# GlassyWing/yolo_deepsort

Measured on AMD Instinct MI355X. Metric: end-to-end frames/sec (detect+ReID+assoc), 608x608, higher is better.
Workload: dtype f16x3

## Files before the change

yolo_deepsort_amd/csrc/conv_f16x3.hip:

```cpp
#include "conv_common.h"

#include <map>
#include <mutex>

#include <math.h>
#include <string.h>

namespace yds {


constexpr int ROWB = 144;
__device__ __forceinline__ void split4(const f32x4 &v, h4 &hi, h4 &lo) {
#pragma unroll
    for (int c = 0; c < 4; ++c) {
        float xs = v[c] * A_SCALE;
        _Float16 h = (_Float16)xs;
        hi[c] = h;
        lo[c] = (_Float16)((xs - (float)h) * LO_SCALE);
    }
}

template <int BM, int BN, int ACT, int RES, int AIN>
__global__ __launch_bounds__(256, 2) void conv_igemm_f16x3(ConvKernelArgs p) {
    fp16_saturate_on();
    constexpr int WM = 2, WN = 2;
    constexpr int TM = BM / WM / 32, TN = BN / WN / 32;
    constexpr int A_ROWS = BM / 32, B_ROWS = BN / 32;
    extern __shared__ __attribute__((aligned(16))) char smem16[];
    char *As = smem16;
    char *Bs = smem16 + 2 * BM * ROWB;

    const int tid = threadIdx.x;
    const int lane = tid & 63, wave = __builtin_amdgcn_readfirstlane(tid >> 6);
    const int wm = wave / WN, wn = wave % WN;
    int m0, n0;
    {
        int tm, tn;
        if (!tile_of_block(p, tm, tn)) return;
        m0 = tm * BM;
        n0 = tn * BN;
    }
    const int cq = tid & 7;
    const int r0 = tid >> 3;

    int a_base[A_ROWS], a_iy[A_ROWS], a_ix[A_ROWS];
    const int HoWo = p.Ho * p.Wo;
#pragma unroll
    for (int i = 0; i < A_ROWS; ++i) {
        int m = m0 + r0 + 32 * i;
        if (m < p.M) {
            int img = m / HoWo, rem = m - img * HoWo;
            int oy = rem / p.Wo, ox = rem - oy * p.Wo;
            a_iy[i] = oy * p.stride - p.pad;
            a_ix[i] = ox * p.stride - p.pad;
            a_base[i] = ((img * p.H + a_iy[i]) * p.W + a_ix[i]) * p.ldx;
        } else {
            a_iy[i] = -(1 << 28);
            a_ix[i] = 0;
            a_base[i] = 0;
        }
    }
    int kk = cq * 4, kh = 0, kw = 0, kc = AIN == FMT_H16 ? 0 : kk;
    if (AIN != FMT_H16)
        while (kc >= p.Cin) { kc -= p.Cin; if (++kw == p.ksize) { kw = 0; ++kh; } }
    unsigned w_off[B_ROWS];
#pragma unroll
    for (int i = 0; i < B_ROWS; ++i) w_off[i] = (unsigned)min(n0 + r0 + 32 * i, p.Cout - 1) * (unsigned)p.Kpad * 4u + cq * 16;
    const char *w_bytes = reinterpret_cast<const char *>(p.w), *x_bytes = reinterpret_cast<const char *>(p.x);

    f32x4 a_reg[A_ROWS], b_reg[B_ROWS];
    unsigned a_ok = 0, a_off[A_ROWS], tap_ok = 0;
    int kt_load = 0;
    auto set_tap = [&]() {
        tap_ok = 0;
#pragma unroll
        for (int i = 0; i < A_ROWS; ++i) {
            int iy = a_iy[i] + kh, ix = a_ix[i] + kw;
            bool ok = (unsigned)iy < (unsigned)p.H && (unsigned)ix < (unsigned)p.W;
            tap_ok |= (ok ? 1u : 0u) << i;
            a_off[i] = ok ? (unsigned)(a_base[i] + (kh * p.W + kw) * p.ldx + cq * 4) * 4u : cq * 16u;
        }
    };
    if (AIN == FMT_H16) set_tap();
    auto load_tiles = [&]() {
        if (AIN == FMT_H16) {
            a_ok = tap_ok;
            const char *xg = x_bytes + (size_t)kc * 4;
#pragma unroll
            for (int i = 0; i < A_ROWS; ++i) a_reg[i] = *reinterpret_cast<const f32x4 *>(xg + a_off[i]);
        } else {
            const int tap_off = (kh * p.W + kw) * p.ldx + kc;
            const bool k_ok = kk < p.K;
            a_ok = 0;
#pragma unroll
            for (int i = 0; i < A_ROWS; ++i) {
                int iy = a_iy[i] + kh, ix = a_ix[i] + kw;
                bool ok = k_ok && (unsigned)iy < (unsigned)p.H && (unsigned)ix < (unsigned)p.W;
                a_ok |= (ok ? 1u : 0u) << i;
                a_reg[i] = *reinterpret_cast<const f32x4 *>(p.x + (ok ? a_base[i] + tap_off : 0));
            }
        }
        const char *wg = w_bytes + (size_t)kt_load * 128;
#pragma unroll
        for (int i = 0; i < B_ROWS; ++i) b_reg[i] = *reinterpret_cast<const f32x4 *>(wg + w_off[i]);
    };
    auto advance_k = [&]() {
        ++kt_load;
        kk += 32;
        kc += 32;
        if (AIN == FMT_H16) {
            if (kc >= p.Cin) { kc = 0; if (++kw == p.ksize) { kw = 0; ++kh; } set_tap(); }
        } else {
            while (kc >= p.Cin) { kc -= p.Cin; if (++kw == p.ksize) { kw = 0; ++kh; } }
        }
    };
    auto store_tiles = [&](int buf) {
        char *a = As + buf * BM * ROWB, *b = Bs + buf * BN * ROWB;
#pragma unroll
        for (int i = 0; i < A_ROWS; ++i) {
            f32x4 v = a_reg[i];
            if (!((a_ok >> i) & 1u)) v = f32x4{0, 0, 0, 0};
            if (AIN == FMT_H16) {
                *reinterpret_cast<f32x4 *>(a + (r0 + 32 * i) * ROWB + cq * 16) = v;
            } else {
                h4 hi, lo;
                split4(v, hi, lo);
                char *row = a + (r0 + 32 * i) * ROWB + cq * 8;
                *reinterpret_cast<h4 *>(row) = hi;
                *reinterpret_cast<h4 *>(row + 64) = lo;
            }
        }
#pragma unroll
        for (int i = 0; i < B_ROWS; ++i) *reinterpret_cast<f32x4 *>(b + (r0 + 32 * i) * ROWB + cq * 16) = b_reg[i];
    };

    f32x16 acc1[TM][TN], acc2[TM][TN];
#pragma unroll
    for (int i = 0; i < TM; ++i)
#pragma unroll
        for (int j = 0; j < TN; ++j)
#pragma unroll
            for (int e = 0; e < 16; ++e) { acc1[i][j][e] = 0.f; acc2[i][j][e] = 0.f; }

    const int nk = p.Kpad / 32;
    load_tiles();
    store_tiles(0);
    if (STAGGER && ((blockIdx.x >> 8) & 1)) __builtin_amdgcn_s_sleep(STAGGER / 4);
    __syncthreads();

    const int frag_off = (lane & 31) * ROWB + (lane >> 5) * 16;
    const char *a_lds = As + wm * (BM / WM) * ROWB + frag_off;
    const char *b_lds = Bs + wn * (BN / WN) * ROWB + frag_off;
    for (int kt = 0; kt < nk; ++kt) {
        const int cur = kt & 1;
        const bool more = kt + 1 < nk;
        if (more) { advance_k(); load_tiles(); }
        const char *a = a_lds + cur * BM * ROWB, *b = b_lds + cur * BN * ROWB;
#pragma unroll
        for (int s = 0; s < 2; ++s) {
            h8 ah[TM], al[TM], bh[TN], bl[TN];
#pragma unroll
            for (int i = 0; i < TM; ++i) {
                ah[i] = *reinterpret_cast<const h8 *>(a + i * 32 * ROWB + s * 32);
                al[i] = *reinterpret_cast<const h8 *>(a + i * 32 * ROWB + s * 32 + 64);
            }
#pragma unroll
            for (int j = 0; j < TN; ++j) {
                bh[j] = *reinterpret_cast<const h8 *>(b + j * 32 * ROWB + s * 32);
                bl[j] = *reinterpret_cast<const h8 *>(b + j * 32 * ROWB + s * 32 + 64);
            }
#pragma unroll
            for (int i = 0; i < TM; ++i)
#pragma unroll
                for (int j = 0; j < TN; ++j) {
                    acc1[i][j] = __builtin_amdgcn_mfma_f32_32x32x16_f16(ah[i], bh[j], acc1[i][j], 0, 0, 0);
                    acc2[i][j] = __builtin_amdgcn_mfma_f32_32x32x16_f16(ah[i], bl[j], acc2[i][j], 0, 0, 0);
                    acc2[i][j] = __builtin_amdgcn_mfma_f32_32x32x16_f16(al[i], bh[j], acc2[i][j], 0, 0, 0);
                }
        }
        if (more) store_tiles(cur ^ 1);
        __syncthreads();
    }
#pragma unroll
    for (int i = 0; i < TM; ++i)
#pragma unroll
        for (int j = 0; j < TN; ++j)
#pragma unroll
            for (int e = 0; e < 16; ++e) acc1[i][j][e] = (acc1[i][j][e] + acc2[i][j][e] * (1.f / LO_SCALE)) * (1.f / A_SCALE);
    static_assert(BM * (BN + 4) * 4 <= 2 * (BM + BN) * ROWB, "whole-tile epilogue staging must fit the main-loop LDS");
    conv_epilogue<BM, BN, WM, WN, ACT, RES, BM / WM / 32, BN / WN / 32, 256, true>(p, acc1, reinterpret_cast<float *>(smem16), m0, n0, tid);
}


constexpr int ZERO_PAGE_BYTES = 64 * 1024;

constexpr size_t dma_smem_bytes(int BM, int BN, int NS) {
    return (size_t)NS * (BM + BN) * 128 > conv_stage_bytes(BM, BN) ? (size_t)NS * (BM + BN) * 128 : conv_stage_bytes(BM, BN);
}
template <int BM, int BN, int WM, int WN, int NS, int ACT, int RES, int TERMS>
__global__ __launch_bounds__(WM * WN * 64, (WM * WN != 4 || dma_smem_bytes(BM, BN, NS) > 80 * 1024) ? 1 : (dma_smem_bytes(BM, BN, NS) <= 53 * 1024 ? 3 : 2))
void conv_igemm_f16x3_dma(ConvKernelArgs p, const char *zero_page) {
    fp16_saturate_on();
    constexpr int NW = WM * WN, NT = NW * 64;
    constexpr int TM = BM / WM / 32, TN = BN / WN / 32;
    constexpr int ROW = 128;
    constexpr int A_BYTES = BM * ROW, STAGE = (BM + BN) * ROW;
    constexpr int A_INST = BM / (8 * NW), B_INST = BN / (8 * NW);
    constexpr int IN = A_INST + B_INST;
    static_assert(NS >= 2 && NS <= 4 && A_INST >= 1 && B_INST >= 1, "ring shape");
    extern __shared__ __attribute__((aligned(16))) char ring[];

    const int tid = threadIdx.x;
    const int lane = tid & 63, wave = __builtin_amdgcn_readfirstlane(tid >> 6);
    const int wm = wave / WN, wn = wave % WN;
    int m0, n0;
    {
        int tm, tn;
        if (!tile_of_block(p, tm, tn)) return;
        m0 = tm * BM;
        n0 = tn * BN;
    }
    const int drow = lane >> 3, dpos = lane & 7;
    int a_base[A_INST], a_iy[A_INST], a_ix[A_INST];
    const char *a_src[A_INST];
    const int HoWo = p.Ho * p.Wo;
#pragma unroll
    for (int q = 0; q < A_INST; ++q) {
        const int row = (q * NW + wave) * 8 + drow;
        const int m = m0 + row;
        if (m < p.M) {
            int img = m / HoWo, rem = m - img * HoWo;
            int oy = rem / p.Wo, ox = rem - oy * p.Wo;
            a_iy[q] = oy * p.stride - p.pad;
            a_ix[q] = ox * p.stride - p.pad;
            a_base[q] = ((img * p.H + a_iy[q]) * p.W + a_ix[q]) * p.ldx;
        } else {
            a_iy[q] = -(1 << 28);
            a_ix[q] = 0;
            a_base[q] = 0;
        }
    }
    constexpr int KC = TERMS == 4 ? 64 : 32;
    const bool xs = TERMS == 4 && p.fmt_x == FMT_F16;
    const int xbpc = xs ? 2 : 4;
    auto src_chunk = [&](int q, bool act) {
        const int c = dpos ^ ((((q * NW + wave) * 8 + drow) >> 1) & 7);
        return ((TERMS == 4 && !(act && xs)) ? ((c >> 2) << 3) + (c & 3) : c) * 16;
    };
    const char *w_src[B_INST];
#pragma unroll
    for (int q = 0; q < B_INST; ++q) {
        const int row = (q * NW + wave) * 8 + drow;
        w_src[q] = reinterpret_cast<const char *>(p.w) + (size_t)min(n0 + row, p.Cout - 1) * p.Kpad * 4 + src_chunk(q, false);
    }
    const int nk_all = p.K / KC;
    int t_begin = 0, nk = nk_all;
    if (gridDim.y > 1) {
        const int per = (nk_all + gridDim.y - 1) / gridDim.y;
        t_begin = blockIdx.y * per;
        nk = max(0, min(nk_all, t_begin + per) - t_begin);
        p.y += (size_t)blockIdx.y * (size_t)p.M * p.ldy;
    }
    const int kcs = p.Cin / KC;
    int kh = (t_begin / kcs) / p.ksize, kw = (t_begin / kcs) % p.ksize, kc = (t_begin % kcs) * KC;
#pragma unroll
    for (int q = 0; q < B_INST; ++q) w_src[q] += (size_t)t_begin * (KC * 4);
    auto set_tap = [&]() {
#pragma unroll
        for (int q = 0; q < A_INST; ++q) {
            int iy = a_iy[q] + kh, ix = a_ix[q] + kw;
            bool ok = (unsigned)iy < (unsigned)p.H && (unsigned)ix < (unsigned)p.W;
            a_src[q] = ok ? reinterpret_cast<const char *>(p.x + (a_base[q] + (kh * p.W + kw) * p.ldx)) + src_chunk(q, true) : zero_page;
        }
    };
    set_tap();
    auto piece = [&](int stage, int q) {
        char *sa = ring + stage * STAGE, *sb = sa + A_BYTES;
        if (q < A_INST) {
            __builtin_amdgcn_global_load_lds((glb_void_t *)(a_src[q] + kc * xbpc), (lds_void_t *)(sa + (q * NW + wave) * 8 * ROW), 16, 0, 0);
        } else {
            const int b = q - A_INST;
            __builtin_amdgcn_global_load_lds((glb_void_t *)w_src[b], (lds_void_t *)(sb + (b * NW + wave) * 8 * ROW), 16, 0, 0);
            w_src[b] += KC * 4;
        }
    };
    auto advance_tile = [&]() {
        kc += KC;
        if (kc >= p.Cin) { kc = 0; if (++kw == p.ksize) { kw = 0; ++kh; } set_tap(); }
    };

    f32x16 acc1[TM][TN], acc2[TM][TN];
#pragma unroll
    for (int i = 0; i < TM; ++i)
#pragma unroll
        for (int j = 0; j < TN; ++j)
#pragma unroll
            for (int e = 0; e < 16; ++e) { acc1[i][j][e] = 0.f; acc2[i][j][e] = 0.f; }

#pragma unroll
    for (int s = 0; s < NS - 1; ++s)
        if (s < nk) {
#pragma unroll
            for (int q = 0; q < IN; ++q) piece(s, q);
            advance_tile();
        }
    if (STAGGER && ((blockIdx.x >> 8) & 1)) __builtin_amdgcn_s_sleep(STAGGER / 4);

    const int swz = (lane >> 1) & 7, kb = lane >> 5;
    const int a_frag = (wm * (BM / WM) + (lane & 31)) * ROW, b_frag = A_BYTES + (wn * (BN / WN) + (lane & 31)) * ROW;
    int pos_hi[2], pos_lo[2];
#pragma unroll
    for (int s = 0; s < 2; ++s) { pos_hi[s] = ((2 * s + kb) ^ swz) * 16; pos_lo[s] = ((4 + 2 * s + kb) ^ swz) * 16; }

    constexpr int NF = 2 * (TM + TN);
    constexpr int NM = 3 * TM * TN;
    h8 fr[2][NF];
    auto frag_read = [&](const char *st, int s, int f) {
        const int which = f / 2, lo = f & 1;
        if (TERMS == 1 && lo) return;
        const int off = which < TM ? a_frag + which * 32 * ROW : b_frag + (which - TM) * 32 * ROW;
        fr[s][f] = *reinterpret_cast<const h8 *>(st + off + (lo ? pos_lo[s] : pos_hi[s]));
    };
    auto mfma = [&](int s, int m) {
        const int ij = m / 3, term = m % 3, i = ij / TN, j = ij % TN;
        if (TERMS == 1 && term != 0) return;
        const h8 ah = fr[s][2 * i], al = fr[s][2 * i + 1], bh = fr[s][2 * (TM + j)], bl = fr[s][2 * (TM + j) + 1];
        if (TERMS == 4) {
            if (term == 0) acc1[i][j] = __builtin_amdgcn_mfma_f32_32x32x16_f16(ah, bh, acc1[i][j], 0, 0, 0);
            else if (term == 1) acc1[i][j] = __builtin_amdgcn_mfma_f32_32x32x16_f16(al, bl, acc1[i][j], 0, 0, 0);
            return;
        }
        if (term == 0) acc1[i][j] = __builtin_amdgcn_mfma_f32_32x32x16_f16(ah, bh, acc1[i][j], 0, 0, 0);
        else if (term == 1) acc2[i][j] = __builtin_amdgcn_mfma_f32_32x32x16_f16(ah, bl, acc2[i][j], 0, 0, 0);
        else acc2[i][j] = __builtin_amdgcn_mfma_f32_32x32x16_f16(al, bh, acc2[i][j], 0, 0, 0);
    };
    constexpr int P0 = IN < NM - 4 ? IN : NM - 4;
    constexpr int F0 = NM - P0 < NF ? NM - P0 : NF;
    static_assert(IN - P0 + NF - F0 <= NM, "not enough MFMA slots for the interleaved memory instructions");
    auto frag_order = [&](int k) {
        if (k < 2) return k;
        if (k < 4) return 2 * TM + (k - 2);
        const int r = k - 4, nb = 2 * (TN - 1);
        return r < nb ? 2 * TM + 2 + r : 2 + (r - nb);
    };
    auto step = [&](int t, auto refill_c) {
        constexpr bool REFILL = decltype(refill_c)::value;
        const char *st = ring + (t % NS) * STAGE;
        const int fill_stage = (t + NS - 1) % NS;
#pragma unroll
        for (int f = 0; f < NF; ++f) frag_read(st, 0, f);
        __builtin_amdgcn_sched_barrier(0);
#pragma unroll
        for (int m = 0; m < NM; ++m) {
            mfma(0, m);
            __builtin_amdgcn_sched_barrier(0);
            if (m < P0) { if (REFILL) piece(fill_stage, m); }
            else if (m - P0 < F0) frag_read(st, 1, frag_order(m - P0));
            __builtin_amdgcn_sched_barrier(0);
        }
#pragma unroll
        for (int m = 0; m < NM; ++m) {
            mfma(1, m);
            __builtin_amdgcn_sched_barrier(0);
            if (m < NF - F0) frag_read(st, 1, frag_order(F0 + m));
            else if (REFILL && P0 + (m - (NF - F0)) < IN) piece(fill_stage, P0 + (m - (NF - F0)));
            __builtin_amdgcn_sched_barrier(0);
        }
        if (REFILL) advance_tile();
    };
    int t = 0;
    for (; t + NS - 1 < nk; ++t) {
        wait_vmcnt<(NS - 2) * IN>();
        __builtin_amdgcn_s_barrier();
        step(t, std::true_type{});
    }
    for (; t < nk; ++t) {
        const int younger = nk - 1 - t;
        if (younger >= 1 && NS >= 3) wait_vmcnt<(NS >= 3 ? IN : 0)>(); else wait_vmcnt<0>();
        __builtin_amdgcn_s_barrier();
        step(t, std::false_type{});
    }
    __syncthreads();
#pragma unroll
    for (int i = 0; i < TM; ++i)
#pragma unroll
        for (int j = 0; j < TN; ++j)
#pragma unroll
            for (int e = 0; e < 16; ++e)
                acc1[i][j][e] = TERMS != 3 ? acc1[i][j][e] * (1.f / A_SCALE) : (acc1[i][j][e] + acc2[i][j][e] * (1.f / LO_SCALE)) * (1.f / A_SCALE);
    conv_epilogue<BM, BN, WM, WN, ACT, RES, TM, TN, NT, true>(p, acc1, reinterpret_cast<float *>(ring), m0, n0, tid);
}

static const char *zero_page_dev() {
    static void *z = nullptr;
    if (!z) {
        YDS_HIP(hipMalloc(&z, ZERO_PAGE_BYTES));
        YDS_HIP(hipMemset(z, 0, ZERO_PAGE_BYTES));
    }
    return static_cast<const char *>(z);
}

template <int BM, int BN, int WM, int WN, int NS> static void launch_cfg_dma(const ConvKernelArgs &k, hipStream_t s) {
    const bool xs = k.fmt_x == FMT_F16;
    if (xs ? (k.terms != 1 || k.Cin % 64) : (k.fmt_x != FMT_H16 || k.Cin % 32)) fail("conv: the LDS-DMA kernel needs a pre-split (H16, or F16 in half mode) input");
    if ((size_t)k.Cin * 4 + 128 > (size_t)ZERO_PAGE_BYTES) fail("conv: %d input channels exceed the zero page of the LDS-DMA kernel", k.Cin);
    auto launch = [&](auto A, auto R, auto terms_c) {
        constexpr int TERMS = decltype(terms_c)::value;
        launch_conv_tiles<conv_igemm_f16x3_dma<BM, BN, WM, WN, NS, A, R, TERMS>>(k, BM, BN, k.ksplit > 1 ? k.ksplit : 1, WM * WN * 64, dma_smem_bytes(BM, BN, NS), s,
                                                                                  zero_page_dev());
    };
    dispatch_act_res(k, [&](auto A, auto R) {
        if (k.terms == 1 && k.Cin % 64 == 0) launch(A, R, std::integral_constant<int, 4>{});
        else if (k.terms == 1) launch(A, R, std::integral_constant<int, 1>{});
        else launch(A, R, std::integral_constant<int, 3>{});
    });
}

__global__ __launch_bounds__(256) void splitk_reduce_kernel(const float *ws, int ksplit, int M, int ldw, ConvKernelArgs p) {
    fp16_saturate_on();
    const int c4 = (p.Cout + 3) / 4;
    const int idx = blockIdx.x * 256 + threadIdx.x;
    if (idx >= M * c4) return;
    const int m = idx / c4, n = (idx - m * c4) * 4;
    float v[4] = {0.f, 0.f, 0.f, 0.f};
    for (int z = 0; z < ksplit; ++z) {
        const float4 t = *reinterpret_cast<const float4 *>(ws + ((size_t)z * M + m) * ldw + n);
        v[0] += t.x; v[1] += t.y; v[2] += t.z; v[3] += t.w;
    }
    float r[4] = {0.f, 0.f, 0.f, 0.f};
    const bool full = n + 3 < p.Cout;
    if (p.res_mode != RES_NONE) {
        const float *rp = p.res + (size_t)m * p.ldr;
        if (p.fmt_r == FMT_H16 || full) load4(rp, n, p.fmt_r, r);
        else for (int k = 0; k < 4; ++k) if (n + k < p.Cout) r[k] = rp[n + k];
    }
#pragma unroll
    for (int k = 0; k < 4; ++k) {
        float o = v[k] + (n + k < p.Cout ? p.bias[n + k] : 0.f);
        if (p.res_mode == RES_BEFORE_ACT) o += r[k];
        o = p.act == ACT_LEAKY ? apply_act<ACT_LEAKY>(o) : p.act == ACT_MISH ? apply_act<ACT_MISH>(o) : p.act == ACT_RELU ? apply_act<ACT_RELU>(o) : o;
        if (p.res_mode == RES_AFTER_ACT) o += r[k];
        v[k] = o;
    }
    float *yp = p.y + (size_t)m * p.ldy;
    if (p.fmt_y == FMT_H16 || full) store4(yp, n, p.fmt_y, v);
    else for (int k = 0; k < 4; ++k) if (n + k < p.Cout) yp[n + k] = v[k];
}

int conv_splitk_factor(const ConvKernelArgs &k, int BM, int BN) {
    const long tiles = (long)((k.M + BM - 1) / BM) * ((k.Cout + BN - 1) / BN);
    const int nk = k.K / 32;
    int s = (int)((512 + tiles - 1) / tiles);
    s = std::min(s, std::min(16, nk / 4));
    return s >= 2 ? s : 1;
}

static float *splitk_workspace(size_t floats, hipStream_t s) {
    static std::mutex mu;
    static std::map<hipStream_t, DevBuf<float>> bufs;
    std::lock_guard<std::mutex> lock(mu);
    DevBuf<float> &b = bufs[s];
    if (b.n < floats) {
        YDS_HIP(hipStreamSynchronize(s));
        b.alloc(floats + floats / 2);
    }
    return b.p;
}

template <int BM, int BN> static void launch_splitk(const ConvKernelArgs &k, hipStream_t s) {
    if (k.fmt_x != FMT_H16 || k.Cin % 32) fail("conv: the split-K LDS-DMA kernel needs a pre-split (H16) input");
    if ((size_t)k.Cout * 4 > (size_t)ZERO_PAGE_BYTES) fail("conv: %d filters exceed the zero page used as the split-K bias", k.Cout);
    const int ksplit = conv_splitk_factor(k, BM, BN);
    if (ksplit < 2) fail("conv: split-K does not apply (the layer already has enough tiles or too few K steps)");
    const int ldw = (k.Cout + 3) / 4 * 4;
    float *ws = splitk_workspace((size_t)ksplit * k.M * ldw, s);
    ConvKernelArgs part = k;
    part.y = ws; part.ldy = ldw; part.fmt_y = FMT_F32;
    part.bias = reinterpret_cast<const float *>(zero_page_dev());
    part.res = nullptr; part.res_mode = RES_NONE; part.fmt_r = FMT_F32; part.act = ACT_LINEAR;
    part.ksplit = ksplit;
    launch_cfg_dma<BM, BN, 2, 2, 2>(part, s);
    const int c4 = (k.Cout + 3) / 4;
    hipLaunchKernelGGL(splitk_reduce_kernel, dim3(((size_t)k.M * c4 + 255) / 256), dim3(256), 0, s, ws, ksplit, k.M, ldw, k);
    YDS_HIP(hipGetLastError());
}

bool conv_splitk_preferred(const ConvKernelArgs &k) {
    if (k.fmt_x != FMT_H16 || k.Cin % 32) return false;
    const long tiles = (long)((k.M + 63) / 64) * ((k.Cout + 127) / 128);
    return tiles <= 128 && k.K / 32 >= 32 && conv_splitk_factor(k, 64, 128) >= 2;
}

bool conv_splitk_applicable(const ConvKernelArgs &k, int tile) {
    if (k.fmt_x != FMT_H16 || k.Cin % 32) return false;
    return tile == 0 ? conv_splitk_factor(k, 64, 128) >= 2 : conv_splitk_factor(k, 128, 128) >= 2;
}

template <int BM, int BN> static void launch_cfg16(const ConvKernelArgs &k, hipStream_t s) {
    if (k.fmt_x == FMT_F16) fail("conv: the register-staged kernel does not read 2-byte (F16) activations");
    constexpr size_t smem = 2ull * (BM + BN) * ROWB;
    dispatch_act_res(k, [&](auto A, auto R) {
        if (k.fmt_x == FMT_H16) launch_conv_tiles<conv_igemm_f16x3<BM, BN, A, R, FMT_H16>>(k, BM, BN, 1, 256, smem, s);
        else launch_conv_tiles<conv_igemm_f16x3<BM, BN, A, R, FMT_F32>>(k, BM, BN, 1, 256, smem, s);
    });
}

void launch_conv_f16x3_staged(ConvKernelArgs k, int tile, hipStream_t s) {
    switch (tile) {
        case 0: launch_cfg16<128, 128>(k, s); break;
        case 1: launch_cfg16<64, 128>(k, s); break;
        case 2: launch_cfg16<128, 64>(k, s); break;
        default: launch_cfg16<64, 64>(k, s); break;
    }
}

void launch_conv_f16x3_dma(ConvKernelArgs k, int tile, hipStream_t s) {
    switch (tile) {
        case 0: launch_cfg_dma<128, 128, 2, 2, 2>(k, s); break;
        case 1: launch_cfg_dma<256, 128, 4, 2, 3>(k, s); break;
        case 2: launch_cfg_dma<128, 256, 2, 4, 3>(k, s); break;
        case 3: launch_cfg_dma<128, 128, 2, 2, 3>(k, s); break;
        case 4: launch_cfg_dma<128, 64, 2, 2, 2>(k, s); break;
        default: launch_cfg_dma<64, 128, 2, 2, 2>(k, s); break;
    }
}

void launch_conv_f16x3_win(ConvKernelArgs k, int tile, hipStream_t s) {
    if (!conv_win_applicable(k)) fail("conv: the window-resident kernel needs a 3x3 stride-1 layer with a pre-split input and W <= 95 (W <= 318 for 32 input channels)");
    if (k.terms == 1) launch_conv_win(k, tile, s);
    else launch_conv_win16(k, tile, s);
}

void launch_conv_f16x3_splitk(ConvKernelArgs k, int tile, hipStream_t s) {
    if (tile == 0) launch_splitk<64, 128>(k, s);
    else launch_splitk<128, 128>(k, s);
}

void pack_weights_f16x3(const float *w, int cout, int kpad, std::vector<uint16_t> &out) {
    out.assign((size_t)cout * kpad * 2, 0);
    for (int o = 0; o < cout; ++o)
        for (int k = 0; k < kpad; ++k) {
            float x = w[(size_t)o * kpad + k];
            if (!(fabsf(x) < 65504.f)) fail("conv: weight %g does not fit the fp16 split (|w| must be < 65504)", (double)x);
            _Float16 h = (_Float16)x;
            _Float16 l = (_Float16)((x - (float)h) * LO_SCALE);
            size_t base = ((size_t)o * (kpad / 32) + k / 32) * 64;
            uint16_t hb, lb;
            memcpy(&hb, &h, 2);
            memcpy(&lb, &l, 2);
            out[base + (k & 31)] = hb;
            out[base + 32 + (k & 31)] = lb;
        }
}

}
```

Baseline: 1649.

## Add 16x16x32 MFMA quadrant-pipelined body for f16x3 LDS-DMA conv kernel

For the three-term split-f16 path on selected tile shapes, this adds an alternative main loop built on 16x16x32 MFMAs in place of 32x32x16. The wave tile is split into quadrants, and the fragment reads and DMA refills are interleaved between quadrant MFMA groups. All NS stages are prefetched and there is one barrier per tile, placed mid-step. The goal is to hide LDS fragment reads and global-to-LDS loads more fully behind MFMA work. It relies on a conv_epilogue16 helper that is not shown here, and it raises register pressure and scheduling complexity.

```diff
diff --git a/yolo_deepsort_amd/csrc/conv_f16x3.hip b/yolo_deepsort_amd/csrc/conv_f16x3.hip
--- a/yolo_deepsort_amd/csrc/conv_f16x3.hip
+++ b/yolo_deepsort_amd/csrc/conv_f16x3.hip
@@ -197,6 +197,20 @@
 constexpr size_t dma_smem_bytes(int BM, int BN, int NS) {
     return (size_t)NS * (BM + BN) * 128 > conv_stage_bytes(BM, BN) ? (size_t)NS * (BM + BN) * 128 : conv_stage_bytes(BM, BN);
 }
+#ifndef YDS_DMA16
+#define YDS_DMA16 -1
+#endif
+constexpr bool dma_body16(int BM, int BN, int NS) {
+    if (YDS_DMA16 >= 0) return YDS_DMA16 != 0;
+    if (BM == 128 && BN == 128 && NS == 2) return true;
+    if (BM == 256 && BN == 128) return true;
+    if (BM == 128 && BN == 256) return true;
+    if (BM == 128 && BN == 128 && NS == 3) return false;
+    if (BM == 128 && BN == 64) return true;
+    if (BM == 64 && BN == 128) return true;
+    return false;
+}
+
 template <int BM, int BN, int WM, int WN, int NS, int ACT, int RES, int TERMS>
 __global__ __launch_bounds__(WM * WN * 64, (WM * WN != 4 || dma_smem_bytes(BM, BN, NS) > 80 * 1024) ? 1 : (dma_smem_bytes(BM, BN, NS) <= 53 * 1024 ? 3 : 2))
 void conv_igemm_f16x3_dma(ConvKernelArgs p, const char *zero_page) {
@@ -289,106 +303,250 @@
         if (kc >= p.Cin) { kc = 0; if (++kw == p.ksize) { kw = 0; ++kh; } set_tap(); }
     };
 
-    f32x16 acc1[TM][TN], acc2[TM][TN];
-#pragma unroll
-    for (int i = 0; i < TM; ++i)
-#pragma unroll
-        for (int j = 0; j < TN; ++j)
-#pragma unroll
-            for (int e = 0; e < 16; ++e) { acc1[i][j][e] = 0.f; acc2[i][j][e] = 0.f; }
-
-#pragma unroll
-    for (int s = 0; s < NS - 1; ++s)
-        if (s < nk) {
-#pragma unroll
-            for (int q = 0; q < IN; ++q) piece(s, q);
-            advance_tile();
-        }
-    if (STAGGER && ((blockIdx.x >> 8) & 1)) __builtin_amdgcn_s_sleep(STAGGER / 4);
-
-    const int swz = (lane >> 1) & 7, kb = lane >> 5;
-    const int a_frag = (wm * (BM / WM) + (lane & 31)) * ROW, b_frag = A_BYTES + (wn * (BN / WN) + (lane & 31)) * ROW;
-    int pos_hi[2], pos_lo[2];
-#pragma unroll
-    for (int s = 0; s < 2; ++s) { pos_hi[s] = ((2 * s + kb) ^ swz) * 16; pos_lo[s] = ((4 + 2 * s + kb) ^ swz) * 16; }
-
-    constexpr int NF = 2 * (TM + TN);
-    constexpr int NM = 3 * TM * TN;
-    h8 fr[2][NF];
-    auto frag_read = [&](const char *st, int s, int f) {
-        const int which = f / 2, lo = f & 1;
-        if (TERMS == 1 && lo) return;
-        const int off = which < TM ? a_frag + which * 32 * ROW : b_frag + (which - TM) * 32 * ROW;
-        fr[s][f] = *reinterpret_cast<const h8 *>(st + off + (lo ? pos_lo[s] : pos_hi[s]));
-    };
-    auto mfma = [&](int s, int m) {
-        const int ij = m / 3, term = m % 3, i = ij / TN, j = ij % TN;
-        if (TERMS == 1 && term != 0) return;
-        const h8 ah = fr[s][2 * i], al = fr[s][2 * i + 1], bh = fr[s][2 * (TM + j)], bl = fr[s][2 * (TM + j) + 1];
-        if (TERMS == 4) {
+    if constexpr (TERMS == 3 && dma_body16(BM, BN, NS)) {
+        constexpr int RW = BM / WM, CW = BN / WN;
+        constexpr int TM16 = RW / 16, TN16 = CW / 16;
+        constexpr int HM = TM16 / 2, HN = TN16 / 2;
+        static_assert(TM16 % 2 == 0 && TN16 % 2 == 0, "the wave tile splits into quadrants");
+        static_assert(NS <= 3, "the drain of the 16x16x32 body counts at most one younger tile");
+        f32x4 acc1[TM16][TN16], acc2[TM16][TN16];
+#pragma unroll
+        for (int i = 0; i < TM16; ++i)
+#pragma unroll
+            for (int j = 0; j < TN16; ++j)
+#pragma unroll
+                for (int e = 0; e < 4; ++e) { acc1[i][j][e] = 0.f; acc2[i][j][e] = 0.f; }
+
+#pragma unroll
+        for (int s = 0; s < NS; ++s)
+            if (s < nk) {
+#pragma unroll
+                for (int q = 0; q < IN; ++q) piece(s, q);
+                advance_tile();
+            }
+
+        const int swz = (lane >> 1) & 7, kq = lane >> 4;
+        const int a_hi = (wm * RW + (lane & 15)) * ROW + ((kq ^ swz) << 4), a_lo = a_hi ^ 64;
+        const int b_hi = A_BYTES + (wn * CW + (lane & 15)) * ROW + ((kq ^ swz) << 4), b_lo = b_hi ^ 64;
+        h8 ah[TM16], al[TM16], bh[TN16], bl[TN16];
+        auto read_a = [&](int stage, int i, bool lo) {
+            const h8 v = *reinterpret_cast<const h8 *>(ring + stage * STAGE + i * 16 * ROW + (lo ? a_lo : a_hi));
+            if (lo) al[i] = v; else ah[i] = v;
+        };
+        auto read_b = [&](int stage, int j, bool lo) {
+            const h8 v = *reinterpret_cast<const h8 *>(ring + stage * STAGE + j * 16 * ROW + (lo ? b_lo : b_hi));
+            if (lo) bl[j] = v; else bh[j] = v;
+        };
+        constexpr int NA = 2 * HM, NB = 2 * HN;
+        constexpr int NMQ = 3 * HM * HN;
+        auto mfma = [&](int qa, int qb, int m) {
+            const int ij = m % (HM * HN), term = m / (HM * HN), i = qa * HM + ij / HN, j = qb * HN + ij % HN;
+            if (term == 0) acc1[i][j] = __builtin_amdgcn_mfma_f32_16x16x32_f16(ah[i], bh[j], acc1[i][j], 0, 0, 0);
+            else if (term == 1) acc2[i][j] = __builtin_amdgcn_mfma_f32_16x16x32_f16(ah[i], bl[j], acc2[i][j], 0, 0, 0);
+            else acc2[i][j] = __builtin_amdgcn_mfma_f32_16x16x32_f16(al[i], bh[j], acc2[i][j], 0, 0, 0);
+        };
+        static_assert(NB + NA <= 2 * NMQ, "Q00 + Q01 hold the fragment reads of H1");
+        constexpr bool NEED_ORDER = IN + HM >= NMQ;
+        constexpr int B_START = IN + NA > NMQ ? IN + NA : NMQ;
+        static_assert(NEED_ORDER ? IN + NA + NB <= 2 * NMQ : B_START + NB <= 2 * NMQ, "Q10 + Q11 hold the DMA pieces and the fragment reads of H0");
+        auto pre_op = [&](int stage, int o) {
+            if (o < HN) read_b(stage, HN + o, false);
+            else if (o < NB) read_b(stage, HN + o - HN, true);
+            else if (o < NB + HM) read_a(stage, HM + o - NB, false);
+            else if (o < NB + NA) read_a(stage, HM + o - NB - HM, true);
+        };
+        auto post_op = [&](int stage, int next, int o, auto refill_c, auto next_c) {
+            constexpr bool REFILL = decltype(refill_c)::value, NEXT = decltype(next_c)::value;
+            if (o < IN) { if (REFILL) piece(stage, o); return; }
+            if (!NEXT) return;
+            const int r = o - IN;
+            if (NEED_ORDER) {
+                if (r < HM) read_a(next, r, false);
+                else if (r < HM + HN) read_b(next, r - HM, false);
+                else if (r < HM + NB) read_b(next, r - HM - HN, true);
+                else if (r < NA + NB) read_a(next, r - HM - NB, true);
+            } else {
+                const int rb = o - B_START;
+                if (r < HM) read_a(next, r, false);
+                else if (r < NA) read_a(next, r - HM, true);
+                else if (rb >= 0 && rb < HN) read_b(next, rb, false);
+                else if (rb >= HN && rb < NB) read_b(next, rb - HN, true);
+            }
+        };
+        auto step_head = [&](int stage) {
+#pragma unroll
+            for (int m = 0; m < NMQ; ++m) {
+                mfma(0, 0, m);
+                __builtin_amdgcn_sched_barrier(0);
+                pre_op(stage, m);
+                __builtin_amdgcn_sched_barrier(0);
+            }
+#pragma unroll
+            for (int m = 0; m < NMQ; ++m) {
+                mfma(0, 1, m);
+                __builtin_amdgcn_sched_barrier(0);
+                pre_op(stage, NMQ + m);
+                __builtin_amdgcn_sched_barrier(0);
+            }
+            asm volatile("s_waitcnt lgkmcnt(0)" ::: "memory");
+        };
+        auto step_tail = [&](int stage, int next, auto refill_c, auto next_c) {
+            __builtin_amdgcn_s_barrier();
+            __builtin_amdgcn_sched_barrier(0);
+#pragma unroll
+            for (int m = 0; m < NMQ; ++m) {
+                mfma(1, 0, m);
+                __builtin_amdgcn_sched_barrier(0);
+                post_op(stage, next, m, refill_c, next_c);
+                __builtin_amdgcn_sched_barrier(0);
+            }
+#pragma unroll
+            for (int m = 0; m < NMQ; ++m) {
+                mfma(1, 1, m);
+                __builtin_amdgcn_sched_barrier(0);
+                post_op(stage, next, NMQ + m, refill_c, next_c);
+                __builtin_amdgcn_sched_barrier(0);
+            }
+            if (decltype(refill_c)::value) advance_tile();
+        };
+
+        if (nk >= 3 && NS >= 3) wait_vmcnt<2 * IN>(); else if (nk >= 2) wait_vmcnt<IN>(); else wait_vmcnt<0>();
+        __builtin_amdgcn_s_barrier();
+#pragma unroll
+        for (int i = 0; i < HM; ++i) { read_a(0, i, false); read_a(0, i, true); }
+#pragma unroll
+        for (int j = 0; j < HN; ++j) { read_b(0, j, false); read_b(0, j, true); }
+        __builtin_amdgcn_sched_barrier(0);
+
+        int t = 0, stage = 0;
+        for (; t + NS < nk; ++t) {
+            const int next = stage + 1 == NS ? 0 : stage + 1;
+            step_head(stage);
+            wait_vmcnt<(NS - 2) * IN>();
+            step_tail(stage, next, std::true_type{}, std::true_type{});
+            stage = next;
+        }
+        for (; t + 1 < nk; ++t) {
+            const int next = stage + 1 == NS ? 0 : stage + 1;
+            step_head(stage);
+            if (NS >= 3 && nk - 2 - t >= 1) wait_vmcnt<(NS >= 3 ? IN : 0)>(); else wait_vmcnt<0>();
+            step_tail(stage, next, std::false_type{}, std::true_type{});
+            stage = next;
+        }
+        if (t < nk) {
+            step_head(stage);
+            step_tail(stage, stage, std::false_type{}, std::false_type{});
+        }
+        __syncthreads();
+#pragma unroll
+        for (int i = 0; i < TM16; ++i)
+#pragma unroll
+            for (int j = 0; j < TN16; ++j)
+#pragma unroll
+                for (int e = 0; e < 4; ++e) acc1[i][j][e] = (acc1[i][j][e] + acc2[i][j][e] * (1.f / LO_SCALE)) * (1.f / A_SCALE);
+        conv_epilogue16<BM, BN, WM, WN, ACT, RES, TM16, TN16, NT, true>(p, acc1, reinterpret_cast<float *>(ring), m0, n0, tid);
+    } else {
+        f32x16 acc1[TM][TN], acc2[TM][TN];
+#pragma unroll
+        for (int i = 0; i < TM; ++i)
+#pragma unroll
+            for (int j = 0; j < TN; ++j)
+#pragma unroll
+                for (int e = 0; e < 16; ++e) { acc1[i][j][e] = 0.f; acc2[i][j][e] = 0.f; }
+
+#pragma unroll
+        for (int s = 0; s < NS - 1; ++s)
+            if (s < nk) {
+#pragma unroll
+                for (int q = 0; q < IN; ++q) piece(s, q);
+                advance_tile();
+            }
+        if (STAGGER && ((blockIdx.x >> 8) & 1)) __builtin_amdgcn_s_sleep(STAGGER / 4);
+
+        const int swz = (lane >> 1) & 7, kb = lane >> 5;
+        const int a_frag = (wm * (BM / WM) + (lane & 31)) * ROW, b_frag = A_BYTES + (wn * (BN / WN) + (lane & 31)) * ROW;
+        int pos_hi[2], pos_lo[2];
+#pragma unroll
+        for (int s = 0; s < 2; ++s) { pos_hi[s] = ((2 * s + kb) ^ swz) * 16; pos_lo[s] = ((4 + 2 * s + kb) ^ swz) * 16; }
+
+        constexpr int NF = 2 * (TM + TN);
+        constexpr int NM = 3 * TM * TN;
+        h8 fr[2][NF];
+        auto frag_read = [&](const char *st, int s, int f) {
+            const int which = f / 2, lo = f & 1;
+            if (TERMS == 1 && lo) return;
+            const int off = which < TM ? a_frag + which * 32 * ROW : b_frag + (which - TM) * 32 * ROW;
+            fr[s][f] = *reinterpret_cast<const h8 *>(st + off + (lo ? pos_lo[s] : pos_hi[s]));
+        };
+        auto mfma = [&](int s, int m) {
+            const int ij = m / 3, term = m % 3, i = ij / TN, j = ij % TN;
+            if (TERMS == 1 && term != 0) return;
+            const h8 ah = fr[s][2 * i], al = fr[s][2 * i + 1], bh = fr[s][2 * (TM + j)], bl = fr[s][2 * (TM + j) + 1];
+            if (TERMS == 4) {
+                if (term == 0) acc1[i][j] = __builtin_amdgcn_mfma_f32_32x32x16_f16(ah, bh, acc1[i][j], 0, 0, 0);
+                else if (term == 1) acc1[i][j] = __builtin_amdgcn_mfma_f32_32x32x16_f16(al, bl, acc1[i][j], 0, 0, 0);
+                return;
+            }
             if (term == 0) acc1[i][j] = __builtin_amdgcn_mfma_f32_32x32x16_f16(ah, bh, acc1[i][j], 0, 0, 0);
-            else if (term == 1) acc1[i][j] = __builtin_amdgcn_mfma_f32_32x32x16_f16(al, bl, acc1[i][j], 0, 0, 0);
-            return;
-        }
-        if (term == 0) acc1[i][j] = __builtin_amdgcn_mfma_f32_32x32x16_f16(ah, bh, acc1[i][j], 0, 0, 0);
-        else if (term == 1) acc2[i][j] = __builtin_amdgcn_mfma_f32_32x32x16_f16(ah, bl, acc2[i][j], 0, 0, 0);
-        else acc2[i][j] = __builtin_amdgcn_mfma_f32_32x32x16_f16(al, bh, acc2[i][j], 0, 0, 0);
-    };
-    constexpr int P0 = IN < NM - 4 ? IN : NM - 4;
-    constexpr int F0 = NM - P0 < NF ? NM - P0 : NF;
-    static_assert(IN - P0 + NF - F0 <= NM, "not enough MFMA slots for the interleaved memory instructions");
-    auto frag_order = [&](int k) {
-        if (k < 2) return k;
-        if (k < 4) return 2 * TM + (k - 2);
-        const int r = k - 4, nb = 2 * (TN - 1);
-        return r < nb ? 2 * TM + 2 + r : 2 + (r - nb);
-    };
-    auto step = [&](int t, auto refill_c) {
-        constexpr bool REFILL = decltype(refill_c)::value;
-        const char *st = ring + (t % NS) * STAGE;
-        const int fill_stage = (t + NS - 1) % NS;
-#pragma unroll
-        for (int f = 0; f < NF; ++f) frag_read(st, 0, f);
-        __builtin_amdgcn_sched_barrier(0);
-#pragma unroll
-        for (int m = 0; m < NM; ++m) {
-            mfma(0, m);
+            else if (term == 1) acc2[i][j] = __builtin_amdgcn_mfma_f32_32x32x16_f16(ah, bl, acc2[i][j], 0, 0, 0);
+            else acc2[i][j] = __builtin_amdgcn_mfma_f32_32x32x16_f16(al, bh, acc2[i][j], 0, 0, 0);
+        };
+        constexpr int P0 = IN < NM - 4 ? IN : NM - 4;
+        constexpr int F0 = NM - P0 < NF ? NM - P0 : NF;
+        static_assert(IN - P0 + NF - F0 <= NM, "not enough MFMA slots for the interleaved memory instructions");
+        auto frag_order = [&](int k) {
+            if (k < 2) return k;
+            if (k < 4) return 2 * TM + (k - 2);
+            const int r = k - 4, nb = 2 * (TN - 1);
+            return r < nb ? 2 * TM + 2 + r : 2 + (r - nb);
+        };
+        auto step = [&](int t, auto refill_c) {
+            constexpr bool REFILL = decltype(refill_c)::value;
+            const char *st = ring + (t % NS) * STAGE;
+            const int fill_stage = (t + NS - 1) % NS;
+#pragma unroll
+            for (int f = 0; f < NF; ++f) frag_read(st, 0, f);
             __builtin_amdgcn_sched_barrier(0);
-            if (m < P0) { if (REFILL) piece(fill_stage, m); }
-            else if (m - P0 < F0) frag_read(st, 1, frag_order(m - P0));
-            __builtin_amdgcn_sched_barrier(0);
-        }
-#pragma unroll
-        for (int m = 0; m < NM; ++m) {
-            mfma(1, m);
-            __builtin_amdgcn_sched_barrier(0);
-            if (m < NF - F0) frag_read(st, 1, frag_order(F0 + m));
-            else if (REFILL && P0 + (m - (NF - F0)) < IN) piece(fill_stage, P0 + (m - (NF - F0)));
-            __builtin_amdgcn_sched_barrier(0);
-        }
-        if (REFILL) advance_tile();
-    };
-    int t = 0;
-    for (; t + NS - 1 < nk; ++t) {
-        wait_vmcnt<(NS - 2) * IN>();
-        __builtin_amdgcn_s_barrier();
-        step(t, std::true_type{});
-    }
-    for (; t < nk; ++t) {
-        const int younger = nk - 1 - t;
-        if (younger >= 1 && NS >= 3) wait_vmcnt<(NS >= 3 ? IN : 0)>(); else wait_vmcnt<0>();
-        __builtin_amdgcn_s_barrier();
-        step(t, std::false_type{});
-    }
-    __syncthreads();
-#pragma unroll
-    for (int i = 0; i < TM; ++i)
-#pragma unroll
-        for (int j = 0; j < TN; ++j)
-#pragma unroll
-            for (int e = 0; e < 16; ++e)
-                acc1[i][j][e] = TERMS != 3 ? acc1[i][j][e] * (1.f / A_SCALE) : (acc1[i][j][e] + acc2[i][j][e] * (1.f / LO_SCALE)) * (1.f / A_SCALE);
-    conv_epilogue<BM, BN, WM, WN, ACT, RES, TM, TN, NT, true>(p, acc1, reinterpret_cast<float *>(ring), m0, n0, tid);
+#pragma unroll
+            for (int m = 0; m < NM; ++m) {
+                mfma(0, m);
+                __builtin_amdgcn_sched_barrier(0);
+                if (m < P0) { if (REFILL) piece(fill_stage, m); }
+                else if (m - P0 < F0) frag_read(st, 1, frag_order(m - P0));
+                __builtin_amdgcn_sched_barrier(0);
+            }
+#pragma unroll
+            for (int m = 0; m < NM; ++m) {
+                mfma(1, m);
+                __builtin_amdgcn_sched_barrier(0);
+                if (m < NF - F0) frag_read(st, 1, frag_order(F0 + m));
+                else if (REFILL && P0 + (m - (NF - F0)) < IN) piece(fill_stage, P0 + (m - (NF - F0)));
+                __builtin_amdgcn_sched_barrier(0);
+            }
+            if (REFILL) advance_tile();
+        };
+        int t = 0;
+        for (; t + NS - 1 < nk; ++t) {
+            wait_vmcnt<(NS - 2) * IN>();
+            __builtin_amdgcn_s_barrier();
+            step(t, std::true_type{});
+        }
+        for (; t < nk; ++t) {
+            const int younger = nk - 1 - t;
+            if (younger >= 1 && NS >= 3) wait_vmcnt<(NS >= 3 ? IN : 0)>(); else wait_vmcnt<0>();
+            __builtin_amdgcn_s_barrier();
+            step(t, std::false_type{});
+        }
+        __syncthreads();
+#pragma unroll
+        for (int i = 0; i < TM; ++i)
+#pragma unroll
+            for (int j = 0; j < TN; ++j)
+#pragma unroll
+                for (int e = 0; e < 16; ++e)
+                    acc1[i][j][e] = TERMS != 3 ? acc1[i][j][e] * (1.f / A_SCALE) : (acc1[i][j][e] + acc2[i][j][e] * (1.f / LO_SCALE)) * (1.f / A_SCALE);
+        conv_epilogue<BM, BN, WM, WN, ACT, RES, TM, TN, NT, true>(p, acc1, reinterpret_cast<float *>(ring), m0, n0, tid);
+    }
 }
 
 static const char *zero_page_dev() {
```

Measured after the change: 1679, median of 6. 1.02x the previous value.
